# SCUT-BIP-Lab/SplatCo

Measured on AMD Instinct MI355X. Metric: rasterizer fwd+bwd Msplats/s @1080p; PSNR-match vs ref, higher is better.
Workload: dtype f32; 1 GPU; cfg1: 1M synthetic Gaussians (seed 0), 1 view 1920x1080 per GPU, GaussianRasterizer forward+backward, colors_precomp + scale/rotation path; gaussians=1000000, image=1920x1080, visible=1000000, parallelism=1 view per GPU (mv sharding)

## Files before the change

splatco_amd/csrc/blend.hip:

```cpp
#include <type_traits>

#include "common.h"

namespace scr {

typedef float v2f __attribute__((ext_vector_type(2)));

#ifdef SCR_BLEND_COUNT
__device__ __forceinline__ void count_sub_blocks(unsigned long long m, unsigned long long (&len)[4]) {
    len[0] += (m & 0x000000000f0f0f0full) != 0ull;
    len[1] += (m & 0x00000000f0f0f0f0ull) != 0ull;
    len[2] += (m & 0x0f0f0f0f00000000ull) != 0ull;
    len[3] += (m & 0xf0f0f0f000000000ull) != 0ull;
}
#define SCR_COUNT_SUB(m) (count_sub_blocks((m), sub_), count_sub_blocks((m), subc_))
#define SCR_COUNT_CHUNK_END(i)                                                                             \
    do {                                                                                                   \
        const unsigned long long a_ = subc_[0] > subc_[1] ? subc_[0] : subc_[1], b_ = subc_[2] > subc_[3] ? subc_[2] : subc_[3]; \
        cnt_[(i)] += a_ > b_ ? a_ : b_;                                                                    \
        subc_[0] = subc_[1] = subc_[2] = subc_[3] = 0;                                                     \
    } while (0)
#define SCR_COUNT_SUB_FLUSH(i_sum, i_max)                                                                  \
    do {                                                                                                   \
        cnt_[(i_sum)] += sub_[0] + sub_[1] + sub_[2] + sub_[3];                                            \
// ... 317 lines not shown
    w = alpha * T;
    s.behind = SAFE ? s.last_alpha * s.d_last + (1.0f - s.last_alpha) * s.behind : s.last_alpha * (s.d_last - s.behind) + s.behind;
    float d = b.z * s.dLp0 + b.w * s.dLp1 + cb * s.dLp2;
    if (AUX) d += z * s.dLd + s.dLa;
    if (SAFE) d = sel(hit, d, 0.0f);
    Y = G * (T * (d - s.behind));
    if (SAFE) Y = sel(hit, Y, 0.0f);
    s.last_alpha = alpha;
    s.d_last = d;
}
__device__ __forceinline__ void group_transmittance(float& T, const float (&om)[4], float (&Tu)[4]) {
#pragma clang fp contract(off)
    const float P = ((om[0] * om[1]) * om[2]) * om[3];
    float r = __builtin_amdgcn_rcpf(P);
    r = __builtin_fmaf(__builtin_fmaf(-P, r, 1.0f), r, r);
    const float q = T * r;
    Tu[3] = __builtin_fmaf(__builtin_fmaf(-q, P, T), r, q);
    Tu[2] = Tu[3] * om[3];
    Tu[1] = Tu[2] * om[2];
    Tu[0] = Tu[1] * om[1];
    T = Tu[3];
}

typedef float f4_t __attribute__((ext_vector_type(4)));
__device__ __forceinline__ void store16_dword_aligned(void* p, float4 v) {
    const f4_t q = {v.x, v.y, v.z, v.w};
    asm volatile("global_store_dwordx4 %0, %1, off" : : "v"(p), "v"(q) : "memory");
}

__device__ __forceinline__ void masked_add4(float4& r, const float4 (&x)[4], const unsigned long long (&c)[4]) {
    unsigned long long keep;
    asm volatile("s_mov_b64 %4, exec\n\t"
                 "s_mov_b64 exec, %5\n\t"
                 "v_add_f32_e32 %0, %0, %9\n\t"
                 "v_add_f32_e32 %1, %1, %10\n\t"
                 "v_add_f32_e32 %2, %2, %11\n\t"
                 "v_add_f32_e32 %3, %3, %12\n\t"
                 "s_mov_b64 exec, %6\n\t"
                 "v_add_f32_e32 %0, %0, %13\n\t"
                 "v_add_f32_e32 %1, %1, %14\n\t"
                 "v_add_f32_e32 %2, %2, %15\n\t"
                 "v_add_f32_e32 %3, %3, %16\n\t"
                 "s_mov_b64 exec, %7\n\t"
                 "v_add_f32_e32 %0, %0, %17\n\t"
                 "v_add_f32_e32 %1, %1, %18\n\t"
                 "v_add_f32_e32 %2, %2, %19\n\t"
                 "v_add_f32_e32 %3, %3, %20\n\t"
                 "s_mov_b64 exec, %8\n\t"
                 "v_add_f32_e32 %0, %0, %21\n\t"
                 "v_add_f32_e32 %1, %1, %22\n\t"
                 "v_add_f32_e32 %2, %2, %23\n\t"
                 "v_add_f32_e32 %3, %3, %24\n\t"
// ... 15 lines not shown
                 "s_mov_b64 exec, %5\n\t"
                 "v_add_f32_e32 %0, %0, %9\n\t"
                 "s_mov_b64 exec, %1"
                 : "+v"(r), "=&s"(keep)
                 : "s"(c[0]), "s"(c[1]), "s"(c[2]), "s"(c[3]), "v"(x[0]), "v"(x[1]), "v"(x[2]), "v"(x[3]));
}

template <bool AUX> struct RecTail { float x; };
template <> struct RecTail<true> { float x, z; };
constexpr int BCH = 64;
constexpr int BWD_MIN_WAVES = 4;
constexpr int ACC_BUFS = 2;

constexpr int BWD_MIN_WAVES_AUX = 3;
template <bool SAFE, bool AUX>
__global__ void __launch_bounds__(256, AUX ? BWD_MIN_WAVES_AUX : BWD_MIN_WAVES)
blend_backward_kernel(int W, int H, int gx, int tiles, const uint32_t* __restrict__ order, const unsigned long long* __restrict__ total,
                      const uint32_t* __restrict__ ranges,
                      const uint32_t* __restrict__ point_list, const uint32_t* __restrict__ gm_index,
                      const uint2* __restrict__ gm_base,
                      const uint8_t* __restrict__ qmask, const float4* __restrict__ rec,
                      const float* __restrict__ bg, const float* __restrict__ final_T,
                      const uint32_t* __restrict__ n_contrib, const float* __restrict__ dL_dpix,
                      GradRec* __restrict__ grad_rec, unsigned long long* __restrict__ cut_key, unsigned long long stamp,
                      uint8_t* __restrict__ has_rec, const float* __restrict__ dL_ddepth, const float* __restrict__ dL_dalpha,
                      float* __restrict__ grad_z) {
    __shared__ float4 st[4][3][BCH + 4];
    __shared__ float4 accA[ACC_BUFS][4][BCH], accB[ACC_BUFS][4][BCH];
    __shared__ float accC[ACC_BUFS][4][BCH];
    __shared__ float accD[ACC_BUFS][4][BCH];
    __shared__ __attribute__((aligned(16))) float tr[4][TR_WORDS];
    __shared__ uint32_t wave_max[4];
    const int t = blend_tile((int)blockIdx.x, tiles, order, total);
    if (t < 0) return;
    const uint32_t lo = ranges[2 * t], n = ranges[2 * t + 1] - lo;
    if (n == 0) return;
    const int wave = threadIdx.x >> 6, lane = threadIdx.x & 63;
    const int qx0 = (t % gx) * TILE + (wave & 1) * 8, qy0 = (t / gx) * TILE + (wave >> 1) * 8;
    const int px = qx0 + (lane >> 3), py = qy0 + (lane & 7);
    const bool inside = px < W && py < H;
    const float pxf = (float)px, pyf = (float)py;
    const float qx0f = (float)qx0, qy0f = (float)qy0;
    const size_t pix = (size_t)py * W + px, hw = (size_t)H * W;
    const uint32_t last = inside ? n_contrib[pix] : 0u;
    PixState ps;
    ps.T = inside ? final_T[pix] : 0.0f;
    ps.dLp0 = ps.dLp1 = ps.dLp2 = 0.0f;
// ... 57 lines not shown

    constexpr int CUT_MIN_ROUNDS = 3;
    const bool cut = nround - 1 - live_top >= CUT_MIN_ROUNDS;
    if (threadIdx.x == 0) {
        unsigned long long ck = ~0ull;
        if (cut) {
            const uint32_t idc = point_list[lo + (uint32_t)(live_top + 1) * BCH];
            ck = ((unsigned long long)__float_as_uint(rec[3 * (size_t)idc + 2].y) << 32) | idc;
            cut_key[tiles] = stamp;
        }
        cut_key[t] = ck;
    }
    const uint32_t tile_x = (uint32_t)(t % gx), tile_y = (uint32_t)(t / gx);
    auto gm_of = [&](uint32_t pos, uint32_t id) -> uint32_t {
        if (gm_index) return gm_index[pos];
        const uint2 b = gm_base[id];
        return b.x + tile_y * b.y + tile_x;
    };
    if (!cut && (AUX || wave < 3))
        for (int ci = nround - 1; ci > live_top; --ci) {
            const uint32_t i = (uint32_t)ci * BCH + lane;
            if (i < n && qmask[lo + i] != 0) {
                const uint32_t gmi = gm_of(lo + i, point_list[lo + i]);
                GradRec& gr = grad_rec[gmi];
                if (wave == 0) store16_dword_aligned(&gr.a, make_float4(0, 0, 0, 0));
                else if (wave == 1) store16_dword_aligned(&gr.b, make_float4(0, 0, 0, 0));
                else if (!AUX || wave == 2) gr.c = 0.0f;
                else grad_z[gmi] = 0.0f;
            }
        }

    uint32_t m_next = 0, id_next = 0, slot_next = 0;
    uint32_t m_cur = 0, slot_cur = 0, id_cur = 0;
    bool sel_cur = false;
    float4 r0 = make_float4(0, 0, 0, 0), r1 = r0;
    RecTail<AUX> r2 = {};
    auto load_meta = [&](int ci, uint32_t& m, uint32_t& id, uint32_t& slot) {
        const uint32_t i = (uint32_t)ci * BCH + lane;
        const bool have = ci >= 0 && i < n;
        m = have ? qmask[lo + i] : 0u;
        id = have ? point_list[lo + i] : 0u;
        slot = have ? gm_of(lo + i, id) : 0u;
    };
    auto gather = [&](int ci, uint32_t m, uint32_t id, uint32_t slot) {
        const uint32_t i = (uint32_t)ci * BCH + lane;
        sel_cur = ((m >> wave) & 1u) && i < wave_last;
        m_cur = m;
        slot_cur = slot;
        id_cur = id;
        if (sel_cur) {
// ... 154 lines not shown
            const uint32_t i = base + lane;
            float4 r = make_float4(0, 0, 0, 0);
            auto part = [&](int w) {
                return wave == 0 ? accA[par][w][lane] : wave == 1 ? accB[par][w][lane]
                                                                  : make_float4(accC[par][w][lane], 0.0f, 0.0f, 0.0f);
            };
            if constexpr (BWD_BATCH_COMBINE) {
                const unsigned long long took[4] = {lanes(((m_this >> 0) & 1u) && i < wmax0), lanes(((m_this >> 1) & 1u) && i < wmax1),
                                                    lanes(((m_this >> 2) & 1u) && i < wmax2), lanes(((m_this >> 3) & 1u) && i < wmax3)};
                if (wave == 2) {
                    const float x[4] = {accC[par][0][lane], accC[par][1][lane], accC[par][2][lane], accC[par][3][lane]};
                    masked_add4(r.x, x, took);
                } else {
                    const float4* const p = wave == 0 ? &accA[par][0][lane] : &accB[par][0][lane];
                    const float4 x[4] = {p[0], p[BCH], p[2 * BCH], p[3 * BCH]};
                    masked_add4(r, x, took);
                }
            } else {
            if (((m_this >> 0) & 1u) && i < wmax0) { const float4 x = part(0); r.x += x.x; r.y += x.y; r.z += x.z; r.w += x.w; }
            if (((m_this >> 1) & 1u) && i < wmax1) { const float4 x = part(1); r.x += x.x; r.y += x.y; r.z += x.z; r.w += x.w; }
            if (((m_this >> 2) & 1u) && i < wmax2) { const float4 x = part(2); r.x += x.x; r.y += x.y; r.z += x.z; r.w += x.w; }
            if (((m_this >> 3) & 1u) && i < wmax3) { const float4 x = part(3); r.x += x.x; r.y += x.y; r.z += x.z; r.w += x.w; }
            }
            GradRec& gr = grad_rec[slot_this];
            if (wave == 0) store16_dword_aligned(&gr.a, r);
            else if (wave == 1) store16_dword_aligned(&gr.b, r);
            else {
                gr.c = r.x;
                if (has_rec) has_rec[id_this] = 1;
            }
        }
        if (AUX && wave == 3 && base + lane < n && m_this != 0) {
            const uint32_t i = base + lane;
            float r = 0.0f;
            if constexpr (BWD_BATCH_COMBINE) {
                const unsigned long long took[4] = {lanes(((m_this >> 0) & 1u) && i < wmax0), lanes(((m_this >> 1) & 1u) && i < wmax1),
                                                    lanes(((m_this >> 2) & 1u) && i < wmax2), lanes(((m_this >> 3) & 1u) && i < wmax3)};
                const float x[4] = {accD[par][0][lane], accD[par][1][lane], accD[par][2][lane], accD[par][3][lane]};
                masked_add4(r, x, took);
            } else {
            if (((m_this >> 0) & 1u) && i < wmax0) r += accD[par][0][lane];
            if (((m_this >> 1) & 1u) && i < wmax1) r += accD[par][1][lane];
            if (((m_this >> 2) & 1u) && i < wmax2) r += accD[par][2][lane];
            if (((m_this >> 3) & 1u) && i < wmax3) r += accD[par][3][lane];
            }
            grad_z[slot_this] = r;
        }
    }
    SCR_COUNT_SUB_FLUSH(14, 15);
    SCR_COUNT_FLUSH(lane);
}
// ... 1 lines not shown
static int blend_slots_per_xcd(const Grid& g) {
    int cnt[NUM_XCD] = {};
    for (int t = 0; t < g.tiles; ++t) ++cnt[xcd_of_tile(t, g.gx)];
    int m = (g.tiles + NUM_XCD - 1) / NUM_XCD;
    for (int q = 0; q < NUM_XCD; ++q) m = cnt[q] > m ? cnt[q] : m;
    return m;
}

void launch_blend_forward(const KSettings& ks, const GeomView& gv, const BinView& bv, const ImgView& iv,
                          float* out_color, float* out_depth, float* out_alpha, bool longest_first, bool safe,
                          hipStream_t st) {
    Grid g(ks.H, ks.W);
    if (longest_first)
        tile_order_kernel<<<NUM_XCD, 1024, 0, st>>>(g.tiles, g.gx, gv.ranges, gv.tile_count, gv.total + 2, gv.total + 4);
    const bool aux = out_depth != nullptr;
    auto kernel = aux ? (safe ? blend_forward_kernel<true, true> : blend_forward_kernel<false, true>)
                      : (safe ? blend_forward_kernel<true, false> : blend_forward_kernel<false, false>);
    kernel<<<(unsigned)blend_slots_per_xcd(g) * NUM_XCD * 4, 64, 0, st>>>(
        ks.W, ks.H, g.gx, g.tiles, gv.tile_count, gv.total, gv.ranges, bv.point_list, bv.qmask, gv.rec, ks.bg, out_color, iv.final_T,
        iv.n_contrib, out_depth, out_alpha);
}

void launch_blend_backward(const KSettings& ks, const GeomView& gv, const BinView& bv, const ImgView& iv,
                           const float* dL_dcolor, const float* dL_ddepth, const float* dL_dalpha, GradRec* grad_rec,
                           float* grad_z, unsigned long long stamp, bool deep, bool flags, bool safe, hipStream_t st) {
    Grid g(ks.H, ks.W);
    const bool gm_from_base = deep;
    if (flags) { ZeroList z; z.add(gv.has_rec, ((size_t)gv.P + 3) / 4 * 4, st); launch_zero(z, st); }
    const bool aux = grad_z != nullptr;
    auto kernel = aux ? (safe ? blend_backward_kernel<true, true> : blend_backward_kernel<false, true>)
                      : (safe ? blend_backward_kernel<true, false> : blend_backward_kernel<false, false>);
    kernel<<<(unsigned)blend_slots_per_xcd(g) * NUM_XCD, 256, 0, st>>>(
        ks.W, ks.H, g.gx, g.tiles, gv.tile_count, gv.total, gv.ranges, bv.point_list, gm_from_base ? nullptr : bv.gm_index, gv.gm_base,
        bv.qmask, gv.rec, ks.bg,
        iv.final_T, iv.n_contrib, dL_dcolor, grad_rec, iv.cut_key, stamp, flags ? gv.has_rec : nullptr, dL_ddepth, dL_dalpha,
        grad_z);
}

}

#ifdef SCR_BLEND_COUNT
extern "C" int scr_tool_blend_counters(unsigned long long* out20, int reset) {
    if (out20 && hipMemcpyFromSymbol(out20, HIP_SYMBOL(scr::g_blend_counters), scr::SCR_NCOUNT * 8) != hipSuccess) return 1;
    if (reset) {
        unsigned long long z[scr::SCR_NCOUNT] = {};
        if (hipMemcpyToSymbol(HIP_SYMBOL(scr::g_blend_counters), z, scr::SCR_NCOUNT * 8) != hipSuccess) return 1;
    }
    return 0;
}
#endif
```

splatco_amd/csrc/capi.hip:

```cpp
#include <stdarg.h>
#include <stdio.h>
#include <string.h>

#include "capi.h"
#include <dlfcn.h>
#include <atomic>
#include <chrono>
#include <map>
#include <mutex>
#include <utility>
#include <vector>
#include <cstring>

using namespace scr;

static thread_local char g_err[512] = "";

namespace {
struct ProfRec { int idx; hipEvent_t a, b; };
unsigned g_prof_mask = 0;
unsigned g_prof_stride = 1;
unsigned g_prof_seen[32] = {};
std::vector<ProfRec> g_prof_recs;
std::vector<hipEvent_t> g_prof_pool;
// ... 314 lines not shown
    SCR_MARK_FN;
    if (check_settings(settings)) return 1;
    if (P < 0) return fail("P < 0");
    const bool camera = dL_dviewmatrix || dL_dprojmatrix || dL_dcampos;
    if (P == 0) {
        if (dL_dviewmatrix) HIP_TRY(hipMemsetAsync(dL_dviewmatrix, 0, 16 * sizeof(float), (hipStream_t)stream));
        if (dL_dprojmatrix) HIP_TRY(hipMemsetAsync(dL_dprojmatrix, 0, 16 * sizeof(float), (hipStream_t)stream));
        if (dL_dcampos) HIP_TRY(hipMemsetAsync(dL_dcampos, 0, 3 * sizeof(float), (hipStream_t)stream));
        return 0;
    }
    if (check_plan_flags(plan_flags)) return 1;
    if (!geom_buf || !binning_buf || !image_buf || !dL_dcolor || !scratch) return fail("NULL buffer");
    if (!means3D || !radii || !dL_dmeans3D || !dL_dmeans2D || !dL_dopacity) return fail("NULL argument");
    if (shs ? !dL_dsh : !dL_dcolors) return fail("colour gradient output missing");
    if (cov3D_precomp ? !dL_dcov3D : !(dL_dscales && dL_drotations && scales && rotations))
        return fail("covariance gradient output missing");
    hipStream_t st = (hipStream_t)stream;
    KSettings ks = ksettings(settings);
    GeomView gv = geom_view(geom_buf, P, ks.H, ks.W);
    BinView bv = bin_view((void*)binning_buf, I, 0);
    ImgView iv = img_view(image_buf, ks.H, ks.W);
    static std::atomic<unsigned long long> stamp_counter{0x5ca1ab1e00000000ull};
    const unsigned long long stamp = ++stamp_counter;
    float* const grad_z = (I > 0 && (dL_ddepth || dL_dalpha)) ? (float*)((char*)scratch + grad_rec_bytes(I)) : nullptr;
    float* const cam_partials = camera ? (float*)((char*)scratch + grad_rec_bytes(I) + grad_z_bytes(I)) : nullptr;
    if (settings->debug) {
        unsigned long long dev_flags = 0;
        HIP_TRY(hipMemcpyAsync(&dev_flags, gv.total + 3, 8, hipMemcpyDeviceToHost, st));
        HIP_TRY(hipStreamSynchronize(st));
        if ((long long)dev_flags != (long long)plan_flags)
            return fail("plan_flags %lld passed to scr_backward, but the forward pass of this geom_buf raised %llu", (long long)plan_flags, dev_flags);
    }
    if (I > 0) {
        launch_zero_far_records(P, gv, (GradRec*)scratch, grad_z, st);
        CHECK_LAUNCH("zero_far_records_kernel", settings->debug, st);
        { ProfScope ps_(SCR_PROF_BLEND_BACKWARD, st);
          launch_blend_backward(ks, gv, bv, iv, dL_dcolor, dL_ddepth, dL_dalpha, (GradRec*)scratch, grad_z, stamp, deep_lists(I, Grid(ks.H, ks.W).tiles),
                                record_flags(I, Grid(ks.H, ks.W).tiles), (plan_flags & SCR_PLAN_NONFINITE_COLOUR) != 0, st); }
        CHECK_LAUNCH("blend_backward_kernel", settings->debug, st);
    }
    { ProfScope ps_(SCR_PROF_PREPROCESS_BACKWARD, st);
      launch_preprocess_backward(P, M, means3D, scales, rotations, cov3D_precomp, shs, ks, radii, gv, bv,
                                 (const GradRec*)scratch, grad_z, iv.cut_key, stamp, record_flags(I, Grid(ks.H, ks.W).tiles), dL_dmeans3D, dL_dmeans2D, shs ? nullptr : dL_dcolors,
                                 shs ? dL_dsh : nullptr, dL_dopacity, cov3D_precomp ? nullptr : dL_dscales,
                                 cov3D_precomp ? nullptr : dL_drotations, cov3D_precomp ? dL_dcov3D : nullptr, cam_partials,
                                 (plan_flags & SCR_PLAN_ANTIALIASED) != 0, st); }
    CHECK_LAUNCH("preprocess_backward_kernel", settings->debug, st);
    if (camera) {
        launch_camera_grad_finish(P, cam_partials, dL_dviewmatrix, dL_dprojmatrix, dL_dcampos, st);
        CHECK_LAUNCH("camera_grad_finish_kernel", settings->debug, st);
    }
    return 0;
}

int scr_debug_force_deep_lists(int mode) {
    if (mode < -1 || mode > 1) return fail("scr_debug_force_deep_lists: -1 (automatic), 0 or 1");
    scr::g_force_deep_lists = mode;
    return 0;
}

int scr_debug_get(int which, int64_t P, int64_t I, int32_t H, int32_t W, const void* geom_buf,
                  const void* binning_buf, const void* image_buf, void* out, void* stream) {
    SCR_MARK_FN;
    hipStream_t st = (hipStream_t)stream;
    Grid g(H, W);
    const void* src = nullptr;
// ... 97 lines not shown
```

splatco_amd/csrc/common.h:

```cpp
#pragma once
#include <hip/hip_runtime.h>
#include <stdint.h>

#include "../../include/splatco_raster.h"

namespace scr {

__host__ __device__ __forceinline__ uint32_t sat_add_u32(uint32_t a, uint32_t b) {
    const uint32_t s = a + b;
    return s < a ? 0xFFFFFFFFu : s;
}


constexpr int TILE = SCR_TILE;
constexpr int TILE_PIX = TILE * TILE;
constexpr int WAVE = 64;
constexpr int NUM_XCD = 8;
constexpr int PRE_BLOCK = 256;
constexpr int BIN_THREADS = 1024;
constexpr int BIN_ROUNDS = 4;
constexpr int BIN_GPW = BIN_THREADS * BIN_ROUNDS;
constexpr int LDS_HIST_MAX_TILES = 40000;
constexpr int ID_BITS = 28;
constexpr int WG_SORT_MAX = 8192;
constexpr int REC_F = 12;
constexpr int GRAD_F = 9;

inline __host__ __device__ size_t align_up(size_t x, size_t a = 256) { return (x + a - 1) / a * a; }

struct Grid {
    int W, H, gx, gy, tiles;
    __host__ __device__ Grid(int H_, int W_)
        : W(W_), H(H_), gx((W_ + TILE - 1) / TILE), gy((H_ + TILE - 1) / TILE), tiles(gx * gy) {}
};

struct GeomView {
    float4* rec;
    uint32_t* tiles_touched;
    uint32_t* point_offsets;
    uint8_t* clamped;
    uint2* gm_base;
    uint32_t* live_bits;
    uint8_t* has_rec;
    uint32_t* block_sums;
    uint32_t* tile_count;
    uint32_t* ranges;
    uint32_t* cursor;
    int64_t P;
    unsigned long long* total;
// ... 39 lines not shown
    uint32_t* point_list;
    uint32_t* gm_index;
    uint8_t* qmask;
    unsigned long long* keys2;
    size_t bytes;
};

inline __host__ BinView bin_view(void* base, int64_t I, int64_t max_tile_instances) {
    char* p = (char*)base;
    size_t off = 0;
    BinView v;
    auto take = [&](size_t n) { char* q = p ? p + off : nullptr; off += align_up(n); return q; };
    size_t n = (size_t)(I > 0 ? I : 1);
    v.keys = (unsigned long long*)take(n * 8);
    v.point_list = (uint32_t*)take(n * 4);
    v.gm_index = (uint32_t*)take(n * 4);
    v.qmask = (uint8_t*)take(n);
    const bool merge = max_tile_instances > WG_SORT_MAX;
    v.keys2 = merge ? (unsigned long long*)take(n * 8) : nullptr;
    v.bytes = off;
    return v;
}

struct __attribute__((packed, aligned(4))) GradQuad { float x, y, z, w; };
struct __attribute__((packed, aligned(4))) GradRec { GradQuad a, b; float c; };
static_assert(sizeof(GradRec) == 36, "36-byte gradient records");
inline __host__ size_t grad_rec_bytes(int64_t I) { return align_up((size_t)(I > 0 ? I : 1) * sizeof(GradRec)); }
inline __host__ size_t grad_z_bytes(int64_t I) { return align_up((size_t)(I > 0 ? I : 1) * sizeof(float)); }

struct ImgView {
    float* final_T;
    uint32_t* n_contrib;
    unsigned long long* cut_key;
    size_t bytes;
};

inline __host__ ImgView img_view(void* base, int H, int W) {
    char* p = (char*)base;
    size_t off = 0;
    ImgView v;
    auto take = [&](size_t n) { char* q = p ? p + off : nullptr; off += align_up(n); return q; };
    v.final_T = (float*)take((size_t)H * W * 4);
    v.n_contrib = (uint32_t*)take((size_t)H * W * 4);
    v.cut_key = (unsigned long long*)take((size_t)Grid(H, W).tiles * 8 + 8);
    v.bytes = off;
    return v;
}

struct KSettings {
    int H, W;
// ... 103 lines not shown
        const float v = __builtin_amdgcn_fmed3f(sy[hx], dyl[hy], dyh[hy]);
        const float t1 = bcx[hx] * v, t2 = f.c * v * v;
        const float qv = qx[hx] + t1 + t2, magv = qx[hx] + fabsf(t1) + t2;
        const float u = __builtin_amdgcn_fmed3f(sx[hy], dxl[hx], dxh[hx]);
        const float s1 = bcy[hy] * u, s2 = f.a * u * u;
        const float qh = qy[hy] + s1 + s2, magh = qy[hy] + fabsf(s1) + s2;
        const bool far = qv > __builtin_fmaf(1.0e-5f, magv, f.thr) && qh > __builtin_fmaf(1.0e-5f, magh, f.thr);
        if (!far) mask |= 1u << q;
    }
    return mask;
}
__device__ inline uint32_t quadrant_mask(float4 r0, float4 r1, int tile_x0, int tile_y0) { return box_mask4<8>(r0, r1, tile_x0, tile_y0); }


struct ZeroList {
    static constexpr int MAX = 20;
    void* p[MAX];
    unsigned long long n[MAX];
    int count = 0;
    bool full() const { return count >= MAX; }
    void add(void* ptr, size_t bytes, hipStream_t st);
};
void launch_zero(const ZeroList& z, hipStream_t st);
void launch_zero_far_records(int64_t P, const GeomView& gv, GradRec* grad_rec, float* grad_z, hipStream_t st);
inline void ZeroList::add(void* ptr, size_t bytes, hipStream_t st) {
    if (!ptr || !bytes) return;
    if (full()) { launch_zero(*this, st); count = 0; }
    p[count] = ptr;
    n[count] = bytes;
    ++count;
}

void allow_dynamic_lds(const void* kernel, size_t bytes);

void launch_filter(int64_t P, const float* means3D, const float* scales, const float* rotations,
                   const float* cov3D, const KSettings& ks, int32_t* radii, hipStream_t st);
void launch_mark_visible(int64_t P, const float* means3D, const float* view, uint8_t* out, hipStream_t st);
void launch_preprocess(int64_t P, int M, const float* means3D, const float* scales, const float* rotations,
                       const float* cov3D, const float* opacities, const float* shs, const float* colors,
                       const KSettings& ks, const GeomView& gv, int32_t* radii, bool antialiased, hipStream_t st);
void launch_plan_scans(int64_t P, const KSettings& ks, const GeomView& gv, unsigned long long* mailbox,
                       unsigned long long seq, hipStream_t st);
void launch_scatter(int64_t P, const KSettings& ks, const GeomView& gv, const BinView& bv, unsigned long long cap_instances,
                    hipStream_t st);
void launch_tile_sort(const KSettings& ks, const GeomView& gv, const BinView& bv, int64_t max_tile_instances,
                      bool with_gm_index, hipStream_t st);
void launch_blend_forward(const KSettings& ks, const GeomView& gv, const BinView& bv, const ImgView& iv,
                          float* out_color, float* out_depth, float* out_alpha, bool longest_first, bool safe,
                          hipStream_t st);
void launch_blend_backward(const KSettings& ks, const GeomView& gv, const BinView& bv, const ImgView& iv,
                           const float* dL_dcolor, const float* dL_ddepth, const float* dL_dalpha, GradRec* grad_rec,
                           float* grad_z, unsigned long long stamp, bool deep, bool flags, bool safe, hipStream_t st);
void launch_preprocess_backward(int64_t P, int M, const float* means3D, const float* scales,
                                const float* rotations, const float* cov3D, const float* shs,
                                const KSettings& ks, const int32_t* radii, const GeomView& gv,
                                const BinView& bv, const GradRec* grad_rec, const float* grad_z,
                                const unsigned long long* cut_key, unsigned long long stamp, bool deep, float* dL_dmeans3D,
                                float* dL_dmeans2D, float* dL_dcolors, float* dL_dsh, float* dL_dopacity,
                                float* dL_dscales, float* dL_drotations, float* dL_dcov3D, float* cam_partials,
                                bool antialiased, hipStream_t st);
size_t camera_partials_bytes(int64_t P);
void launch_camera_grad_finish(int64_t P, const float* cam_partials, float* dL_dview, float* dL_dproj, float* dL_dcampos,
                               hipStream_t st);

constexpr int NL_DP = 80;

}
```

splatco_amd/csrc/preprocess.hip:

```cpp
#include "wg.h"

namespace scr {

struct Proj {
    float t[3];
    float hx, hy, hw;
    float cov[6];
    float txc, tyc;
    bool clx, cly;
    float T[2][3];
    float a, b, c;
    float a0, c0;
};

__device__ __forceinline__ void xform3(const float* __restrict__ M, float x, float y, float z, int i,
                                       float& out) {
    out = ((M[i] * x + M[4 + i] * y) + M[8 + i] * z) + M[12 + i];
}

__device__ __forceinline__ void rotmat(const float q[4], float R[3][3]) {
    float r = q[0], x = q[1], y = q[2], z = q[3];
    R[0][0] = 1.0f - 2.0f * (y * y + z * z);
    R[0][1] = 2.0f * (x * y - r * z);
    R[0][2] = 2.0f * (x * z + r * y);
// ... 267 lines not shown
        block_sums[blockIdx.x] = tot;
    }
    if (LDS_HIST)
        for (int t = threadIdx.x; t < tiles; t += BIN_THREADS) {
            const uint32_t c = hist[t];
            if (c) atomicAdd(&tile_count[t], c);
        }
}

constexpr int CAM_VALUES = 27, CAM_ROW = 32;
__device__ __forceinline__ void cam_workgroup_sum(float (&v)[CAM_VALUES], float* __restrict__ row) {
    __shared__ float wave_part[(PRE_BLOCK / WAVE) * CAM_VALUES];
    wg_wave_parts<PRE_BLOCK / WAVE>(v, wave_part);
    if (threadIdx.x < CAM_ROW) {
        float tot = 0.0f;
        if (threadIdx.x < CAM_VALUES) {
#pragma unroll
            for (int w = 0; w < PRE_BLOCK / WAVE; ++w) tot += wave_part[w * CAM_VALUES + threadIdx.x];
        }
        row[threadIdx.x] = tot;
    }
}

template <bool AUX, bool POSE, bool AA>
__global__ void __launch_bounds__(PRE_BLOCK, 1)
preprocess_backward_kernel(int64_t P, int M, const float* __restrict__ means3D,
                           const float* __restrict__ scales, const float* __restrict__ rotations,
                           const float* __restrict__ cov3D, const float* __restrict__ shs, KSettings ks,
                           const int32_t* __restrict__ radii, const uint32_t* __restrict__ tiles_touched,
                           const uint32_t* __restrict__ point_offsets, const uint32_t* __restrict__ live_bits,
                           const uint8_t* __restrict__ has_rec, const uint8_t* __restrict__ clamped,
                           const float4* __restrict__ rec, const GradRec* __restrict__ grad_rec,
                           const unsigned long long* __restrict__ cut_key, unsigned long long stamp, int tiles,
                           float* __restrict__ dL_dmeans3D, float* __restrict__ dL_dmeans2D,
                           float* __restrict__ dL_dcolors, float* __restrict__ dL_dsh,
                           float* __restrict__ dL_dopacity, float* __restrict__ dL_dscales,
                           float* __restrict__ dL_drotations, float* __restrict__ dL_dcov3D,
                           const float* __restrict__ grad_z, float* __restrict__ cam_partials,
                           const unsigned long long* __restrict__ plan_word) {
    const bool aa_fwd = (plan_word[0] & (unsigned long long)SCR_PLAN_ANTIALIASED) != 0ull;
    int64_t i = (int64_t)blockIdx.x * PRE_BLOCK + threadIdx.x;
    bool inb = true;
    if (POSE) {
        inb = i < P;
        if (!inb) i = P - 1;
    } else if (i >= P) return;
    float cg[POSE ? CAM_VALUES : 1] = {};
    float gm[3] = {0, 0, 0}, gm2[3] = {0, 0, 0}, gcol[3] = {0, 0, 0}, gop = 0, gs[3] = {0, 0, 0},
          gq[4] = {0, 0, 0, 0}, g6[6] = {0, 0, 0, 0, 0, 0};
    bool vis = radii[i] > 0;
    if (POSE && !inb) vis = false;
    if (has_rec && !has_rec[i]) vis = false;
    const float4 r2 = rec[3 * i + 2];
    Proj ps;
    Foot ft;
    if (vis) vis = project(i, means3D, scales, rotations, cov3D, ks, ps, ft);
    if (vis) {
        uint32_t n = tiles_touched[i];
        uint32_t off = point_offsets[i] - n;
        float sx = 0, sy = 0, sxx = 0, sxy = 0, syy = 0;
        float sz = 0;
        const GradRec* gr = grad_rec + off;
        const float* gz = AUX ? grad_z + off : nullptr;
        const unsigned long long mykey = ((unsigned long long)__float_as_uint(r2.y) << 32) | (uint32_t)i;
        const uint32_t rlo = __float_as_uint(r2.z), rhi = __float_as_uint(r2.w);
        const int gxt = (ks.W + TILE - 1) / TILE, rx0 = (int)(rlo & 0xffffu), rx1 = (int)(rhi & 0xffffu);
        int tcx = rx0, tcy = (int)(rlo >> 16);
        const uint32_t lbits = live_bits[i];
        uint32_t kwalk = 0;
        auto next_tile = [&](bool& live) {
            const int t = tcy * gxt + tcx;
            live = ((lbits >> (kwalk & 31u)) & 1u) != 0u;
            ++kwalk;
            if (++tcx == rx1) { tcx = rx0; ++tcy; }
            return t;
        };
        auto add = [&](const GradRec& q, bool ok) {
            sx += ok ? q.a.x : 0.0f; sy += ok ? q.a.y : 0.0f; sxx += ok ? q.a.z : 0.0f; sxy += ok ? q.a.w : 0.0f;
            syy += ok ? q.b.x : 0.0f; gop += ok ? q.b.y : 0.0f; gcol[0] += ok ? q.b.z : 0.0f; gcol[1] += ok ? q.b.w : 0.0f;
            gcol[2] += ok ? q.c : 0.0f;
        };
        auto addz = [&](float z, bool ok) { sz += ok ? z : 0.0f; };
#define SCR_PB_SRC(live_, p_) (p_)
        uint32_t k = 0;
        const uint32_t nb = n < 32u ? n : 32u;
        const bool any_cut = cut_key[tiles] == stamp;
        if (any_cut) {
            for (; k + 4 <= nb; k += 4) {
                GradRec q[4];
                float z[4] = {0, 0, 0, 0};
                unsigned long long ck[4];
                bool live[4];
#pragma unroll
                for (int j = 0; j < 4; ++j) {
                    ck[j] = cut_key[next_tile(live[j])];
                    q[j] = *SCR_PB_SRC(live[j], gr + k + j);
                    if (AUX) z[j] = gz[k + j];
                }
#pragma unroll
                for (int j = 0; j < 4; ++j) {
                    add(q[j], live[j] && mykey < ck[j]);
                    if (AUX) addz(z[j], live[j] && mykey < ck[j]);
                }
            }
            for (; k < nb; ++k) {
                bool live;
                const unsigned long long ck = cut_key[next_tile(live)];
                const GradRec q = *SCR_PB_SRC(live, gr + k);
                add(q, live && mykey < ck);
                if (AUX) addz(gz[k], live && mykey < ck);
            }
        } else {
            for (; k + 4 <= nb; k += 4) {
                GradRec q[4];
                float z[4] = {0, 0, 0, 0};
                bool live[4];
#pragma unroll
                for (int j = 0; j < 4; ++j) {
                    next_tile(live[j]);
                    q[j] = *SCR_PB_SRC(live[j], gr + k + j);
                    if (AUX) z[j] = gz[k + j];
                }
#pragma unroll
                for (int j = 0; j < 4; ++j) {
                    add(q[j], live[j]);
                    if (AUX) addz(z[j], live[j]);
                }
            }
            for (; k < nb; ++k) {
                bool live;
                next_tile(live);
                add(*SCR_PB_SRC(live, gr + k), live);
                if (AUX) addz(gz[k], live);
            }
        }
        for (; k < n; ++k) {
            add(gr[k], true);
            if (AUX) addz(gz[k], true);
        }
        const float4 ra = rec[3 * i], rb = rec[3 * i + 1];
        const float cA = ra.z, cB = ra.w, cC = rb.x, op = rb.y;
        gop = gop != 0.0f ? gop / op : 0.0f;
        const float gmx = 2.0f * cA * sx + cB * sy, gmy = 2.0f * cC * sy + cB * sx;
        const float gQxx = -0.5f * sxx, gQxy = -sxy, gQyy = -0.5f * syy;
        const float* V = ks.view;
        const float* Pm = ks.proj;
        float a = ps.a, b = ps.b, c = ps.c;
        float det = a * c - b * b;
        float d2 = 1.0f / (det * det);
        float dL_da = d2 * (-c * c * gQxx + b * c * gQxy - b * b * gQyy);
        float dL_db = d2 * (2.0f * b * c * gQxx - (det + 2.0f * b * b) * gQxy + 2.0f * a * b * gQyy);
        float dL_dc = d2 * (-b * b * gQxx + a * b * gQxy - a * a * gQyy);
        if (AA && aa_fwd) {
            float r;
            const float h = aa_factor(ps, det, r);
            if (r > AA_FLOOR) {
                const float o = op / h;
                const float gr = gop * o / (2.0f * h);
                const float det0 = ps.a0 * ps.c0 - b * b;
                dL_da += gr * ((ps.c0 * det - det0 * c) * d2);
// ... 271 lines not shown

void launch_mark_visible(int64_t P, const float* means3D, const float* view, uint8_t* out, hipStream_t st) {
    if (P <= 0) return;
    mark_visible_kernel<<<nblk(P, 256), 256, 0, st>>>(P, means3D, view, out);
}

void launch_preprocess(int64_t P, int M, const float* means3D, const float* scales, const float* rotations,
                       const float* cov3D, const float* opacities, const float* shs, const float* colors,
                       const KSettings& ks, const GeomView& gv, int32_t* radii, bool antialiased, hipStream_t st) {
    if (P <= 0) return;
    Grid g(ks.H, ks.W);
    const bool lds = g.tiles <= LDS_HIST_MAX_TILES;
    auto kernel = lds ? (antialiased ? preprocess_kernel<true, true> : preprocess_kernel<true, false>)
                      : (antialiased ? preprocess_kernel<false, true> : preprocess_kernel<false, false>);
    if (lds) allow_dynamic_lds((const void*)kernel, LDS_HIST_MAX_TILES * 4);
    kernel<<<nblk(P, BIN_GPW), BIN_THREADS, lds ? (size_t)g.tiles * 4 : 0, st>>>(
        P, M, means3D, scales, rotations, cov3D, opacities, shs, colors, ks, g.tiles, gv.rec, gv.tiles_touched,
        shs ? gv.clamped : nullptr, gv.block_sums, gv.tile_count, radii, gv.total + 3);
}

void launch_preprocess_backward(int64_t P, int M, const float* means3D, const float* scales,
                                const float* rotations, const float* cov3D, const float* shs,
                                const KSettings& ks, const int32_t* radii, const GeomView& gv,
                                const BinView& bv, const GradRec* grad_rec, const float* grad_z,
                                const unsigned long long* cut_key, unsigned long long stamp, bool deep, float* dL_dmeans3D,
                                float* dL_dmeans2D, float* dL_dcolors, float* dL_dsh, float* dL_dopacity,
                                float* dL_dscales, float* dL_drotations, float* dL_dcov3D, float* cam_partials,
                                bool antialiased, hipStream_t st) {
    if (P <= 0) return;
    auto kernel = cam_partials ? (grad_z ? preprocess_backward_kernel<true, true, false> : preprocess_backward_kernel<false, true, false>)
                               : (grad_z ? preprocess_backward_kernel<true, false, false> : preprocess_backward_kernel<false, false, false>);
    if (antialiased)
        kernel = cam_partials ? (grad_z ? preprocess_backward_kernel<true, true, true> : preprocess_backward_kernel<false, true, true>)
                              : (grad_z ? preprocess_backward_kernel<true, false, true> : preprocess_backward_kernel<false, false, true>);
    kernel<<<nblk(P, PRE_BLOCK), PRE_BLOCK, 0, st>>>(
        P, M, means3D, scales, rotations, cov3D, shs, ks, radii, gv.tiles_touched, gv.point_offsets, gv.live_bits,
        deep ? gv.has_rec : nullptr, gv.clamped, gv.rec, grad_rec, cut_key, stamp, Grid(ks.H, ks.W).tiles, dL_dmeans3D, dL_dmeans2D, dL_dcolors, dL_dsh, dL_dopacity,
        dL_dscales, dL_drotations, dL_dcov3D, grad_z, cam_partials, gv.total + 3);
}

size_t camera_partials_bytes(int64_t P) { return align_up((size_t)(P > 0 ? nblk(P, PRE_BLOCK) : 1) * CAM_ROW * sizeof(float)); }

void launch_camera_grad_finish(int64_t P, const float* cam_partials, float* dL_dview, float* dL_dproj, float* dL_dcampos,
                               hipStream_t st) {
    camera_grad_finish_kernel<<<1, CAM_FINISH_THREADS, 0, st>>>(P > 0 ? (int64_t)nblk(P, PRE_BLOCK) : 0, cam_partials, dL_dview,
                                                                 dL_dproj, dL_dcampos);
}

__global__ void __launch_bounds__(256) zero_far_records_kernel(int64_t P, const unsigned long long* __restrict__ total,
                                                               const uint32_t* __restrict__ tiles_touched,
                                                               const uint32_t* __restrict__ point_offsets, uint32_t* __restrict__ rec_words,
                                                               float* __restrict__ grad_z) {
    if ((total[3] & (unsigned long long)SCR_PLAN_LARGE_RECTS) == 0ull) return;
    const int lane = threadIdx.x & 63;
    for (int64_t base = (int64_t)blockIdx.x * 256 + (threadIdx.x & ~63); base < P; base += (int64_t)gridDim.x * 256) {
        const int64_t i = base + lane;
        const uint32_t n = i < P ? tiles_touched[i] : 0u;
        const uint32_t end = (i < P && n > 32u) ? point_offsets[i] : 0u;
        unsigned long long big = lanes(n > 32u);
        while (big) {
            const int src = __builtin_ctzll(big);
            big &= big - 1;
            const uint32_t n_s = (uint32_t)__shfl((int)n, src, WAVE), end_s = (uint32_t)__shfl((int)end, src, WAVE);
            const size_t w0 = (size_t)(end_s - n_s + 32u) * GRAD_F, w1 = (size_t)end_s * GRAD_F;
            for (size_t w = w0 + lane; w < w1; w += WAVE) rec_words[w] = 0u;
            if (grad_z)
                for (size_t w = (size_t)(end_s - n_s + 32u) + lane; w < (size_t)end_s; w += WAVE) grad_z[w] = 0.0f;
        }
    }
}
void launch_zero_far_records(int64_t P, const GeomView& gv, GradRec* grad_rec, float* grad_z, hipStream_t st) {
    if (P <= 0) return;
    const int64_t want = (P + 255) / 256;
    zero_far_records_kernel<<<(unsigned)(want < 2048 ? want : 2048), 256, 0, st>>>(P, gv.total, gv.tiles_touched, gv.point_offsets, (uint32_t*)grad_rec, grad_z);
}

__global__ void __launch_bounds__(256) zero_list_kernel(ZeroList z) {
    const unsigned long long bytes = z.n[blockIdx.y];
    char* base = (char*)z.p[blockIdx.y];
    const unsigned long long lo = (unsigned long long)blockIdx.x * 16384ull;
    if (lo >= bytes) return;
    const unsigned long long hi = lo + 16384ull < bytes ? lo + 16384ull : bytes;
    if (((uintptr_t)base & 15) == 0) {
        for (unsigned long long o = lo + 16ull * threadIdx.x; o + 16 <= hi; o += 16ull * 256) *(float4*)(base + o) = make_float4(0, 0, 0, 0);
        for (unsigned long long o = lo + ((hi - lo) & ~15ull) + 4ull * threadIdx.x; o < hi; o += 4ull * 256) *(uint32_t*)(base + o) = 0u;
    } else {
        for (unsigned long long o = lo + 4ull * threadIdx.x; o < hi; o += 4ull * 256) *(uint32_t*)(base + o) = 0u;
    }
}
void launch_zero(const ZeroList& z, hipStream_t st) {
    if (z.count <= 0) return;
    unsigned long long mx = 0;
    for (int i = 0; i < z.count; ++i) mx = z.n[i] > mx ? z.n[i] : mx;
    zero_list_kernel<<<dim3((unsigned)((mx + 16383) / 16384), (unsigned)z.count), 256, 0, st>>>(z);
}

}
// ... 1 lines not shown
```

Before: 1121 Msplats/s.

## Split packed 36-byte gradient records into separate SoA planes

```diff
diff --git a/splatco_amd/csrc/blend.hip b/splatco_amd/csrc/blend.hip
--- a/splatco_amd/csrc/blend.hip
+++ b/splatco_amd/csrc/blend.hip
@@ -363,12 +363,6 @@
     T = Tu[3];
 }
 
-typedef float f4_t __attribute__((ext_vector_type(4)));
-__device__ __forceinline__ void store16_dword_aligned(void* p, float4 v) {
-    const f4_t q = {v.x, v.y, v.z, v.w};
-    asm volatile("global_store_dwordx4 %0, %1, off" : : "v"(p), "v"(q) : "memory");
-}
-
 __device__ __forceinline__ void masked_add4(float4& r, const float4 (&x)[4], const unsigned long long (&c)[4]) {
     unsigned long long keep;
     asm volatile("s_mov_b64 %4, exec\n\t"
@@ -430,7 +424,8 @@
                       const uint8_t* __restrict__ qmask, const float4* __restrict__ rec,
                       const float* __restrict__ bg, const float* __restrict__ final_T,
                       const uint32_t* __restrict__ n_contrib, const float* __restrict__ dL_dpix,
-                      GradRec* __restrict__ grad_rec, unsigned long long* __restrict__ cut_key, unsigned long long stamp,
+                      float4* __restrict__ rec_a, float4* __restrict__ rec_b, float* __restrict__ rec_c,
+                      unsigned long long* __restrict__ cut_key, unsigned long long stamp,
                       uint8_t* __restrict__ has_rec, const float* __restrict__ dL_ddepth, const float* __restrict__ dL_dalpha,
                       float* __restrict__ grad_z) {
     __shared__ float4 st[4][3][BCH + 4];
@@ -534,10 +529,9 @@
             const uint32_t i = (uint32_t)ci * BCH + lane;
             if (i < n && qmask[lo + i] != 0) {
                 const uint32_t gmi = gm_of(lo + i, point_list[lo + i]);
-                GradRec& gr = grad_rec[gmi];
-                if (wave == 0) store16_dword_aligned(&gr.a, make_float4(0, 0, 0, 0));
-                else if (wave == 1) store16_dword_aligned(&gr.b, make_float4(0, 0, 0, 0));
-                else if (!AUX || wave == 2) gr.c = 0.0f;
+                if (wave == 0) rec_a[gmi] = make_float4(0, 0, 0, 0);
+                else if (wave == 1) rec_b[gmi] = make_float4(0, 0, 0, 0);
+                else if (!AUX || wave == 2) rec_c[gmi] = 0.0f;
                 else grad_z[gmi] = 0.0f;
             }
         }
@@ -738,11 +732,10 @@
             if (((m_this >> 2) & 1u) && i < wmax2) { const float4 x = part(2); r.x += x.x; r.y += x.y; r.z += x.z; r.w += x.w; }
             if (((m_this >> 3) & 1u) && i < wmax3) { const float4 x = part(3); r.x += x.x; r.y += x.y; r.z += x.z; r.w += x.w; }
             }
-            GradRec& gr = grad_rec[slot_this];
-            if (wave == 0) store16_dword_aligned(&gr.a, r);
-            else if (wave == 1) store16_dword_aligned(&gr.b, r);
+            if (wave == 0) rec_a[slot_this] = r;
+            else if (wave == 1) rec_b[slot_this] = r;
             else {
-                gr.c = r.x;
+                rec_c[slot_this] = r.x;
                 if (has_rec) has_rec[id_this] = 1;
             }
         }
@@ -790,7 +783,7 @@
 }
 
 void launch_blend_backward(const KSettings& ks, const GeomView& gv, const BinView& bv, const ImgView& iv,
-                           const float* dL_dcolor, const float* dL_ddepth, const float* dL_dalpha, GradRec* grad_rec,
+                           const float* dL_dcolor, const float* dL_ddepth, const float* dL_dalpha, const GradRec& grad_rec,
                            float* grad_z, unsigned long long stamp, bool deep, bool flags, bool safe, hipStream_t st) {
     Grid g(ks.H, ks.W);
     const bool gm_from_base = deep;
@@ -801,7 +794,7 @@
     kernel<<<(unsigned)blend_slots_per_xcd(g) * NUM_XCD, 256, 0, st>>>(
         ks.W, ks.H, g.gx, g.tiles, gv.tile_count, gv.total, gv.ranges, bv.point_list, gm_from_base ? nullptr : bv.gm_index, gv.gm_base,
         bv.qmask, gv.rec, ks.bg,
-        iv.final_T, iv.n_contrib, dL_dcolor, grad_rec, iv.cut_key, stamp, flags ? gv.has_rec : nullptr, dL_ddepth, dL_dalpha,
+        iv.final_T, iv.n_contrib, dL_dcolor, grad_rec.a, grad_rec.b, grad_rec.c, iv.cut_key, stamp, flags ? gv.has_rec : nullptr, dL_ddepth, dL_dalpha,
         grad_z);
 }
 
diff --git a/splatco_amd/csrc/capi.hip b/splatco_amd/csrc/capi.hip
--- a/splatco_amd/csrc/capi.hip
+++ b/splatco_amd/csrc/capi.hip
@@ -360,6 +360,8 @@
     ImgView iv = img_view(image_buf, ks.H, ks.W);
     static std::atomic<unsigned long long> stamp_counter{0x5ca1ab1e00000000ull};
     const unsigned long long stamp = ++stamp_counter;
+    if ((uintptr_t)scratch & 15u) return fail("scratch is not 16-byte aligned");
+    const GradRec grad_rec = grad_rec_view(scratch, I);
     float* const grad_z = (I > 0 && (dL_ddepth || dL_dalpha)) ? (float*)((char*)scratch + grad_rec_bytes(I)) : nullptr;
     float* const cam_partials = camera ? (float*)((char*)scratch + grad_rec_bytes(I) + grad_z_bytes(I)) : nullptr;
     if (settings->debug) {
@@ -370,16 +372,16 @@
             return fail("plan_flags %lld passed to scr_backward, but the forward pass of this geom_buf raised %llu", (long long)plan_flags, dev_flags);
     }
     if (I > 0) {
-        launch_zero_far_records(P, gv, (GradRec*)scratch, grad_z, st);
+        launch_zero_far_records(P, gv, grad_rec, grad_z, st);
         CHECK_LAUNCH("zero_far_records_kernel", settings->debug, st);
         { ProfScope ps_(SCR_PROF_BLEND_BACKWARD, st);
-          launch_blend_backward(ks, gv, bv, iv, dL_dcolor, dL_ddepth, dL_dalpha, (GradRec*)scratch, grad_z, stamp, deep_lists(I, Grid(ks.H, ks.W).tiles),
+          launch_blend_backward(ks, gv, bv, iv, dL_dcolor, dL_ddepth, dL_dalpha, grad_rec, grad_z, stamp, deep_lists(I, Grid(ks.H, ks.W).tiles),
                                 record_flags(I, Grid(ks.H, ks.W).tiles), (plan_flags & SCR_PLAN_NONFINITE_COLOUR) != 0, st); }
         CHECK_LAUNCH("blend_backward_kernel", settings->debug, st);
     }
     { ProfScope ps_(SCR_PROF_PREPROCESS_BACKWARD, st);
       launch_preprocess_backward(P, M, means3D, scales, rotations, cov3D_precomp, shs, ks, radii, gv, bv,
-                                 (const GradRec*)scratch, grad_z, iv.cut_key, stamp, record_flags(I, Grid(ks.H, ks.W).tiles), dL_dmeans3D, dL_dmeans2D, shs ? nullptr : dL_dcolors,
+                                 grad_rec, grad_z, iv.cut_key, stamp, record_flags(I, Grid(ks.H, ks.W).tiles), dL_dmeans3D, dL_dmeans2D, shs ? nullptr : dL_dcolors,
                                  shs ? dL_dsh : nullptr, dL_dopacity, cov3D_precomp ? nullptr : dL_dscales,
                                  cov3D_precomp ? nullptr : dL_drotations, cov3D_precomp ? dL_dcov3D : nullptr, cam_partials,
                                  (plan_flags & SCR_PLAN_ANTIALIASED) != 0, st); }
diff --git a/splatco_amd/csrc/common.h b/splatco_amd/csrc/common.h
--- a/splatco_amd/csrc/common.h
+++ b/splatco_amd/csrc/common.h
@@ -24,7 +24,6 @@
 constexpr int ID_BITS = 28;
 constexpr int WG_SORT_MAX = 8192;
 constexpr int REC_F = 12;
-constexpr int GRAD_F = 9;
 
 inline __host__ __device__ size_t align_up(size_t x, size_t a = 256) { return (x + a - 1) / a * a; }
 
@@ -110,10 +109,14 @@
     return v;
 }
 
-struct __attribute__((packed, aligned(4))) GradQuad { float x, y, z, w; };
-struct __attribute__((packed, aligned(4))) GradRec { GradQuad a, b; float c; };
-static_assert(sizeof(GradRec) == 36, "36-byte gradient records");
-inline __host__ size_t grad_rec_bytes(int64_t I) { return align_up((size_t)(I > 0 ? I : 1) * sizeof(GradRec)); }
+struct GradRec { float4* a; float4* b; float* c; };
+inline __host__ size_t grad_plane_bytes(int64_t I, size_t elem) { return align_up((size_t)(I > 0 ? I : 1) * elem); }
+inline __host__ size_t grad_rec_bytes(int64_t I) { return 2 * grad_plane_bytes(I, sizeof(float4)) + grad_plane_bytes(I, sizeof(float)); }
+inline __host__ GradRec grad_rec_view(void* base, int64_t I) {
+    char* p = (char*)base;
+    const size_t q = grad_plane_bytes(I, sizeof(float4));
+    return GradRec{(float4*)p, (float4*)(p + q), (float*)(p + 2 * q)};
+}
 inline __host__ size_t grad_z_bytes(int64_t I) { return align_up((size_t)(I > 0 ? I : 1) * sizeof(float)); }
 
 struct ImgView {
@@ -263,7 +266,7 @@
     void add(void* ptr, size_t bytes, hipStream_t st);
 };
 void launch_zero(const ZeroList& z, hipStream_t st);
-void launch_zero_far_records(int64_t P, const GeomView& gv, GradRec* grad_rec, float* grad_z, hipStream_t st);
+void launch_zero_far_records(int64_t P, const GeomView& gv, const GradRec& grad_rec, float* grad_z, hipStream_t st);
 inline void ZeroList::add(void* ptr, size_t bytes, hipStream_t st) {
     if (!ptr || !bytes) return;
     if (full()) { launch_zero(*this, st); count = 0; }
@@ -290,12 +293,12 @@
                           float* out_color, float* out_depth, float* out_alpha, bool longest_first, bool safe,
                           hipStream_t st);
 void launch_blend_backward(const KSettings& ks, const GeomView& gv, const BinView& bv, const ImgView& iv,
-                           const float* dL_dcolor, const float* dL_ddepth, const float* dL_dalpha, GradRec* grad_rec,
+                           const float* dL_dcolor, const float* dL_ddepth, const float* dL_dalpha, const GradRec& grad_rec,
                            float* grad_z, unsigned long long stamp, bool deep, bool flags, bool safe, hipStream_t st);
 void launch_preprocess_backward(int64_t P, int M, const float* means3D, const float* scales,
                                 const float* rotations, const float* cov3D, const float* shs,
                                 const KSettings& ks, const int32_t* radii, const GeomView& gv,
-                                const BinView& bv, const GradRec* grad_rec, const float* grad_z,
+                                const BinView& bv, const GradRec& grad_rec, const float* grad_z,
                                 const unsigned long long* cut_key, unsigned long long stamp, bool deep, float* dL_dmeans3D,
                                 float* dL_dmeans2D, float* dL_dcolors, float* dL_dsh, float* dL_dopacity,
                                 float* dL_dscales, float* dL_drotations, float* dL_dcov3D, float* cam_partials,
diff --git a/splatco_amd/csrc/preprocess.hip b/splatco_amd/csrc/preprocess.hip
--- a/splatco_amd/csrc/preprocess.hip
+++ b/splatco_amd/csrc/preprocess.hip
@@ -1,3 +1,4 @@
+#include <type_traits>
 #include "wg.h"
 
 namespace scr {
@@ -313,6 +314,10 @@
     }
 }
 
+#ifndef SCR_PB_FLIGHT
+#define SCR_PB_FLIGHT 4
+#endif
+constexpr int PB_FLIGHT = SCR_PB_FLIGHT;
 template <bool AUX, bool POSE, bool AA>
 __global__ void __launch_bounds__(PRE_BLOCK, 1)
 preprocess_backward_kernel(int64_t P, int M, const float* __restrict__ means3D,
@@ -321,7 +326,8 @@
                            const int32_t* __restrict__ radii, const uint32_t* __restrict__ tiles_touched,
                            const uint32_t* __restrict__ point_offsets, const uint32_t* __restrict__ live_bits,
                            const uint8_t* __restrict__ has_rec, const uint8_t* __restrict__ clamped,
-                           const float4* __restrict__ rec, const GradRec* __restrict__ grad_rec,
+                           const float4* __restrict__ rec, const float4* __restrict__ rec_a,
+                           const float4* __restrict__ rec_b, const float* __restrict__ rec_c,
                            const unsigned long long* __restrict__ cut_key, unsigned long long stamp, int tiles,
                            float* __restrict__ dL_dmeans3D, float* __restrict__ dL_dmeans2D,
                            float* __restrict__ dL_dcolors, float* __restrict__ dL_dsh,
@@ -351,7 +357,9 @@
         uint32_t off = point_offsets[i] - n;
         float sx = 0, sy = 0, sxx = 0, sxy = 0, syy = 0;
         float sz = 0;
-        const GradRec* gr = grad_rec + off;
+        const float4* ga = rec_a + off;
+        const float4* gb = rec_b + off;
+        const float* gc = rec_c + off;
         const float* gz = AUX ? grad_z + off : nullptr;
         const unsigned long long mykey = ((unsigned long long)__float_as_uint(r2.y) << 32) | (uint32_t)i;
         const uint32_t rlo = __float_as_uint(r2.z), rhi = __float_as_uint(r2.w);
@@ -366,67 +374,51 @@
             if (++tcx == rx1) { tcx = rx0; ++tcy; }
             return t;
         };
-        auto add = [&](const GradRec& q, bool ok) {
-            sx += ok ? q.a.x : 0.0f; sy += ok ? q.a.y : 0.0f; sxx += ok ? q.a.z : 0.0f; sxy += ok ? q.a.w : 0.0f;
-            syy += ok ? q.b.x : 0.0f; gop += ok ? q.b.y : 0.0f; gcol[0] += ok ? q.b.z : 0.0f; gcol[1] += ok ? q.b.w : 0.0f;
-            gcol[2] += ok ? q.c : 0.0f;
+        auto add = [&](const float4& qa, const float4& qb, float qc, bool ok) {
+            sx += ok ? qa.x : 0.0f; sy += ok ? qa.y : 0.0f; sxx += ok ? qa.z : 0.0f; sxy += ok ? qa.w : 0.0f;
+            syy += ok ? qb.x : 0.0f; gop += ok ? qb.y : 0.0f; gcol[0] += ok ? qb.z : 0.0f; gcol[1] += ok ? qb.w : 0.0f;
+            gcol[2] += ok ? qc : 0.0f;
         };
         auto addz = [&](float z, bool ok) { sz += ok ? z : 0.0f; };
-#define SCR_PB_SRC(live_, p_) (p_)
         uint32_t k = 0;
         const uint32_t nb = n < 32u ? n : 32u;
         const bool any_cut = cut_key[tiles] == stamp;
+        auto batch = [&](auto cut_c, auto n_c) {
+            constexpr bool CUT = decltype(cut_c)::value;
+            constexpr int N = decltype(n_c)::value;
+            float4 qa[N], qb[N];
+            float qc[N], z[N];
+            unsigned long long ck[N];
+            bool live[N];
+#pragma unroll
+            for (int j = 0; j < N; ++j) {
+                const int t = next_tile(live[j]);
+                ck[j] = CUT ? cut_key[t] : ~0ull;
+                qa[j] = ga[k + j];
+                qb[j] = gb[k + j];
+                qc[j] = gc[k + j];
+                z[j] = AUX ? gz[k + j] : 0.0f;
+            }
+#pragma unroll
+            for (int j = 0; j < N; ++j) {
+                const bool ok = live[j] && (!CUT || mykey < ck[j]);
+                add(qa[j], qb[j], qc[j], ok);
+                if (AUX) addz(z[j], ok);
+            }
+            k += N;
+        };
+        using std::integral_constant;
         if (any_cut) {
-            for (; k + 4 <= nb; k += 4) {
-                GradRec q[4];
-                float z[4] = {0, 0, 0, 0};
-                unsigned long long ck[4];
-                bool live[4];
-#pragma unroll
-                for (int j = 0; j < 4; ++j) {
-                    ck[j] = cut_key[next_tile(live[j])];
-                    q[j] = *SCR_PB_SRC(live[j], gr + k + j);
-                    if (AUX) z[j] = gz[k + j];
-                }
-#pragma unroll
-                for (int j = 0; j < 4; ++j) {
-                    add(q[j], live[j] && mykey < ck[j]);
-                    if (AUX) addz(z[j], live[j] && mykey < ck[j]);
-                }
-            }
-            for (; k < nb; ++k) {
-                bool live;
-                const unsigned long long ck = cut_key[next_tile(live)];
-                const GradRec q = *SCR_PB_SRC(live, gr + k);
-                add(q, live && mykey < ck);
-                if (AUX) addz(gz[k], live && mykey < ck);
-            }
+            while (k + PB_FLIGHT <= nb) batch(integral_constant<bool, true>{}, integral_constant<int, PB_FLIGHT>{});
+            if constexpr (PB_FLIGHT > 4) while (k + 4 <= nb) batch(integral_constant<bool, true>{}, integral_constant<int, 4>{});
+            while (k < nb) batch(integral_constant<bool, true>{}, integral_constant<int, 1>{});
         } else {
-            for (; k + 4 <= nb; k += 4) {
-                GradRec q[4];
-                float z[4] = {0, 0, 0, 0};
-                bool live[4];
-#pragma unroll
-                for (int j = 0; j < 4; ++j) {
-                    next_tile(live[j]);
-                    q[j] = *SCR_PB_SRC(live[j], gr + k + j);
-                    if (AUX) z[j] = gz[k + j];
-                }
-#pragma unroll
-                for (int j = 0; j < 4; ++j) {
-                    add(q[j], live[j]);
-                    if (AUX) addz(z[j], live[j]);
-                }
-            }
-            for (; k < nb; ++k) {
-                bool live;
-                next_tile(live);
-                add(*SCR_PB_SRC(live, gr + k), live);
-                if (AUX) addz(gz[k], live);
-            }
+            while (k + PB_FLIGHT <= nb) batch(integral_constant<bool, false>{}, integral_constant<int, PB_FLIGHT>{});
+            if constexpr (PB_FLIGHT > 4) while (k + 4 <= nb) batch(integral_constant<bool, false>{}, integral_constant<int, 4>{});
+            while (k < nb) batch(integral_constant<bool, false>{}, integral_constant<int, 1>{});
         }
         for (; k < n; ++k) {
-            add(gr[k], true);
+            add(ga[k], gb[k], gc[k], true);
             if (AUX) addz(gz[k], true);
         }
         const float4 ra = rec[3 * i], rb = rec[3 * i + 1];
@@ -744,7 +736,7 @@
 void launch_preprocess_backward(int64_t P, int M, const float* means3D, const float* scales,
                                 const float* rotations, const float* cov3D, const float* shs,
                                 const KSettings& ks, const int32_t* radii, const GeomView& gv,
-                                const BinView& bv, const GradRec* grad_rec, const float* grad_z,
+                                const BinView& bv, const GradRec& grad_rec, const float* grad_z,
                                 const unsigned long long* cut_key, unsigned long long stamp, bool deep, float* dL_dmeans3D,
                                 float* dL_dmeans2D, float* dL_dcolors, float* dL_dsh, float* dL_dopacity,
                                 float* dL_dscales, float* dL_drotations, float* dL_dcov3D, float* cam_partials,
@@ -757,7 +749,7 @@
                               : (grad_z ? preprocess_backward_kernel<true, false, true> : preprocess_backward_kernel<false, false, true>);
     kernel<<<nblk(P, PRE_BLOCK), PRE_BLOCK, 0, st>>>(
         P, M, means3D, scales, rotations, cov3D, shs, ks, radii, gv.tiles_touched, gv.point_offsets, gv.live_bits,
-        deep ? gv.has_rec : nullptr, gv.clamped, gv.rec, grad_rec, cut_key, stamp, Grid(ks.H, ks.W).tiles, dL_dmeans3D, dL_dmeans2D, dL_dcolors, dL_dsh, dL_dopacity,
+        deep ? gv.has_rec : nullptr, gv.clamped, gv.rec, grad_rec.a, grad_rec.b, grad_rec.c, cut_key, stamp, Grid(ks.H, ks.W).tiles, dL_dmeans3D, dL_dmeans2D, dL_dcolors, dL_dsh, dL_dopacity,
         dL_dscales, dL_drotations, dL_dcov3D, grad_z, cam_partials, gv.total + 3);
 }
 
@@ -771,7 +763,8 @@
 
 __global__ void __launch_bounds__(256) zero_far_records_kernel(int64_t P, const unsigned long long* __restrict__ total,
                                                                const uint32_t* __restrict__ tiles_touched,
-                                                               const uint32_t* __restrict__ point_offsets, uint32_t* __restrict__ rec_words,
+                                                               const uint32_t* __restrict__ point_offsets, float4* __restrict__ rec_a,
+                                                               float4* __restrict__ rec_b, float* __restrict__ rec_c,
                                                                float* __restrict__ grad_z) {
     if ((total[3] & (unsigned long long)SCR_PLAN_LARGE_RECTS) == 0ull) return;
     const int lane = threadIdx.x & 63;
@@ -784,17 +777,19 @@
             const int src = __builtin_ctzll(big);
             big &= big - 1;
             const uint32_t n_s = (uint32_t)__shfl((int)n, src, WAVE), end_s = (uint32_t)__shfl((int)end, src, WAVE);
-            const size_t w0 = (size_t)(end_s - n_s + 32u) * GRAD_F, w1 = (size_t)end_s * GRAD_F;
-            for (size_t w = w0 + lane; w < w1; w += WAVE) rec_words[w] = 0u;
-            if (grad_z)
-                for (size_t w = (size_t)(end_s - n_s + 32u) + lane; w < (size_t)end_s; w += WAVE) grad_z[w] = 0.0f;
-        }
-    }
-}
-void launch_zero_far_records(int64_t P, const GeomView& gv, GradRec* grad_rec, float* grad_z, hipStream_t st) {
+            for (size_t w = (size_t)(end_s - n_s + 32u) + lane; w < (size_t)end_s; w += WAVE) {
+                rec_a[w] = make_float4(0, 0, 0, 0);
+                rec_b[w] = make_float4(0, 0, 0, 0);
+                rec_c[w] = 0.0f;
+                if (grad_z) grad_z[w] = 0.0f;
+            }
+        }
+    }
+}
+void launch_zero_far_records(int64_t P, const GeomView& gv, const GradRec& grad_rec, float* grad_z, hipStream_t st) {
     if (P <= 0) return;
     const int64_t want = (P + 255) / 256;
-    zero_far_records_kernel<<<(unsigned)(want < 2048 ? want : 2048), 256, 0, st>>>(P, gv.total, gv.tiles_touched, gv.point_offsets, (uint32_t*)grad_rec, grad_z);
+    zero_far_records_kernel<<<(unsigned)(want < 2048 ? want : 2048), 256, 0, st>>>(P, gv.total, gv.tiles_touched, gv.point_offsets, grad_rec.a, grad_rec.b, grad_rec.c, grad_z);
 }
 
 __global__ void __launch_bounds__(256) zero_list_kernel(ZeroList z) {
```

Result: no change. 1112 Msplats/s (-0.8%).
